# POZAlabs/ComMU-code

Measured on AMD Instinct MI355X. Metric: training tokens/sec at d_model=512 tgt_len=1024, higher is better.
Workload: dtype bf16; 1 GPU; transformer-xl train step L6 D512 H8 DI1024 tgt_len1024 mem_len0 vocab729; global_batch=64, batch_per_gpu=64, batch_chunk=1, seq_len=1024, parallelism=dp1, optimizer=clip1.0+Adam+invsqrt-LR, launch=eager, weights=random init (train.py:291-342)

## Files before the change

commu-code_amd/commu_amd/_lib.py:

```python
from __future__ import annotations

import ctypes as C
import os

_HERE = os.path.dirname(os.path.abspath(__file__))
LIB_PATH = os.path.join(os.path.dirname(_HERE), "lib", "libcommu_hip.so")

c_p = C.c_void_p
c_i = C.c_int
c_f = C.c_float
c_z = C.c_size_t


class AttnDesc(C.Structure):
    _fields_ = [("q", c_p), ("k", c_p), ("v", c_p), ("rd", c_p), ("r_w_bias", c_p), ("r_r_bias", c_p),
                ("reset", c_p), ("ld_qkv", c_i), ("ld_rd", c_i), ("ld_o", c_i), ("T", c_i), ("M", c_i),
                ("B", c_i), ("H", c_i), ("DH", c_i), ("same_length", c_i), ("sshift", c_i), ("scale", c_f),
                ("drop_p", c_f), ("drop_seed", C.c_uint)]


class AttnBwdDesc(C.Structure):
    _fields_ = [("dout", c_p), ("lse", c_p), ("delta", c_p), ("qu2", c_p), ("qv2", c_p), ("dq_ac", c_p),
                ("dk", c_p), ("dv", c_p), ("dsk", c_p), ("du_part", c_p), ("ld_dqkv", c_i), ("ld_dsk", c_i),
                ("du_rows", c_i), ("dsk_wedge", c_i), ("dsk_tiled", c_i), ("p_scratch", c_p), ("o", c_p), ("pf", c_p)]
# ... 36 lines not shown

class DecodeLoopArgs(C.Structure):
    _fields_ = [("struct_bytes", C.c_uint),
                ("logits", c_p), ("wrong", c_p), ("ld", c_i), ("V", c_i), ("B", c_i),
                ("temperature_rows", c_p), ("top_k_rows", c_p), ("top_p_rows", c_p),
                ("temperature", c_f), ("top_k", c_i), ("top_p", c_f),
                ("token", c_p), ("probs_out", c_p), ("logp", c_p), ("seq_logp", c_p), ("ldp", c_i),
                ("state", c_p), ("seq", c_p), ("chord_tok", c_p), ("chord_pos", c_p), ("utable", c_p),
                ("ld_seq", c_i), ("ld_chord", c_i), ("ld_u", c_i), ("max_iters", c_i),
                ("tok", c_p), ("active", c_p), ("keep", c_p), ("draw", c_p), ("uni", c_p), ("trace", c_p), ("ld_trace", c_i),
                ("klen", c_p), ("lmax", c_i),
                ("bias", c_p), ("gram", c_p), ("gram_on", c_p), ("harm", c_p), ("harm_on", c_p),
                ("ld_bias", c_i), ("ld_gram", c_i), ("ld_harm", c_i),
                ("cls_ctl", c_p)]


def struct_args(cls, **fields):
    return cls(struct_bytes=C.sizeof(cls), **fields)


PROTOTYPES = {
    "commu_gemm_nt_bf16": [c_p, c_i, c_p, c_i, c_p, c_i, c_i, c_i, c_i, c_p, c_p, c_i, c_p, c_i, c_i, C.c_uint, c_f, c_f, c_p],
    "commu_gemm_nt_signbits_words": [c_i, c_i, c_i, c_i, c_i, c_i],
    "commu_gemm_nt_ln_bf16": [c_p, c_i, c_p, c_p, c_i, c_f, c_p, c_i, c_p, c_i, c_p, c_i, c_i, c_i, c_i, c_p, c_p, c_i, c_i, c_p],
    "commu_gemm_tn_bf16": [c_p, c_i, c_p, c_i, c_p, c_i, c_z, c_i, c_i, c_i, c_i, c_i, c_p],
    "commu_gemm_nt_bf16_batched": [c_p, c_i, C.c_longlong, c_p, c_i, C.c_longlong, c_p, c_i, C.c_longlong, c_i, c_i,
                                   c_i, c_p, c_i, C.c_longlong, c_i, c_i, c_i, c_i, c_p],
    "commu_gemm_tn_slices": [c_i, c_i, c_i],
    "commu_gemm_tn_bf16_batched": [c_p, c_i, C.c_longlong, c_p, c_i, C.c_longlong, c_p, c_i, c_z, c_i, c_i, c_i, c_i,
                                   c_i, c_i, c_i, c_p],
    "commu_gemm_tn_grouped_slices": [C.POINTER(TnProblem), c_i, c_i],
    "commu_gemm_tn_grouped_slices_budget": [C.POINTER(TnProblem), c_i, c_i, c_i],
    "commu_gemm_tn_bf16_grouped": [C.POINTER(TnProblem), c_i, c_i, c_p, C.c_longlong, c_i, c_p],
    "commu_reduce_slabs2d_f32": [c_p, c_i, C.c_longlong, c_p, c_i, c_i, c_i, c_z, c_i, c_i, c_f, c_p],
    "commu_reduce_slabs_f32": [c_p, c_p, c_z, c_i, c_z, c_i, c_f, c_p],
    "commu_quant_mxfp8": [c_p, c_i, c_p, c_i, c_p, c_i, c_i, c_i, c_p],
    "commu_gemm_nt_mxfp8": [c_p, c_i, c_p, c_i, c_p, c_i, c_p, c_i, c_p, c_i, c_i, c_i, c_i, c_p, c_p, c_i, c_i, C.c_uint, c_f, c_p],
    "commu_reduce_slabs_group_f32": [C.POINTER(ReduceItem), c_i, c_p, c_i, c_z, c_i, c_f, c_p],
    "commu_reduce_slabs_crop_f32": [c_p, c_p, c_i, c_i, c_i, c_i, c_i, c_i, c_i, c_z, c_i, c_f, c_p],
    "commu_embed_fwd": [c_p, c_p, c_p, c_i, c_i, c_i, c_i, c_f, C.c_uint, c_f, c_p],
    "commu_embed_bwd": [c_p, c_p, c_i, c_p, c_i, c_i, c_i, c_f, c_i, C.c_uint, c_f, c_p],
    "commu_embed_bwd_ws_rows": [c_i, c_i],
    "commu_embed_bwd_sorted": [c_p, c_p, c_p, c_i, c_p, c_i, c_i, c_i, c_p, c_f, c_i, C.c_uint, c_f, c_p],
    "commu_posemb_fwd": [c_p, c_p, c_i, c_i, c_i, c_i, C.c_uint, c_f, c_p],
    "commu_layernorm_fwd": [c_p, c_i, c_p, c_p, c_p, c_i, c_p, c_p, c_i, c_i, c_f, c_p, c_i, C.c_uint, c_f, c_p],
    "commu_layernorm_bwd_nblocks": [c_i],
# ... 84 lines not shown
    "commu_embed_f32": [c_p, c_p, c_p, c_i, c_i, c_i, c_f, c_p],
    "commu_posemb_f32": [c_p, c_p, c_i, c_i, c_i, c_i, c_p],
    "commu_relattn_f32": [c_p, c_i, c_p, c_p, C.c_longlong, C.c_longlong, c_p, c_i, c_p, c_p, c_p, c_p, c_p, c_i, c_i, c_i,
                          c_i, c_i, c_i, c_i, c_i, c_f, c_p],
    "commu_decode_kv_append_f32": [c_p, c_i, c_p, c_p, c_p, c_p, c_i, c_i, c_i, c_p],
    "commu_decode_kv_append_ring_f32": [c_p, c_i, c_p, c_p, c_p, c_p, c_i, c_i, c_i, c_p],
    "commu_decode_attn_ring_f32": [c_p, c_i, c_p, c_p, c_p, c_i, c_p, c_p, c_p, c_p, c_i, c_i, c_i, c_i, c_i, c_i, c_f, c_p],
    "commu_gemm_f32": [c_i, c_i, c_p, c_i, c_p, c_i, c_p, c_i, c_i, c_i, c_i, c_p, c_i, c_f, C.c_uint, c_p, c_i, c_i, c_p, c_i,
                       c_p],
    "commu_relattn_fwd_f32": [c_p, c_i, c_p, c_p, c_i, c_p, c_i, c_p, c_p, c_p, c_p, c_i, c_p, c_i, c_i, c_i, c_i, c_i, c_i, c_i,
                              c_f, c_f, C.c_uint, c_p],
    "commu_relattn_bwd_f32": [c_p, c_i, c_p, c_p, c_i, c_p, c_i, c_p, c_p, c_p, c_p, c_i, c_p, c_i, c_p, c_p, c_p, c_i, c_p, c_p,
                              c_p, c_p, c_i, c_p, c_i, c_i, c_i, c_i, c_i, c_i, c_i, c_i, c_f, c_f, C.c_uint, c_p],
    "commu_layernorm_fwd_f32": [c_p, c_i, c_p, c_p, c_p, c_i, c_p, c_p, c_i, c_i, c_f, c_p],
    "commu_layernorm_bwd_f32": [c_p, c_i, c_p, c_i, c_p, c_i, c_p, c_p, c_p, c_p, c_i, c_p, c_i, c_p, c_p, c_i, c_i, c_p],
    "commu_ce_bwd_f32": [c_p, c_i, c_p, c_p, c_p, c_p, c_i, c_i, c_i, c_p],
    "commu_embed_bwd_f32": [c_p, c_p, c_p, c_i, c_p, c_i, c_i, c_f, c_f, C.c_uint, c_p],
    "commu_dropout_f32": [c_p, c_i, c_p, c_i, c_p, c_i, c_i, c_i, c_f, C.c_uint, c_p],
    "commu_hip_version": [],
}
_RESTYPE = {"commu_decode_tail_pack_bytes": C.c_longlong, "commu_attn_pf_bytes": C.c_longlong, "commu_hip_version": C.c_char_p, "commu_attn_p_scratch_elems": C.c_longlong,
            "commu_gemm_nt_signbits_words": C.c_longlong, "commu_pack_batch": C.c_longlong}
_NOCHECK = {"commu_layernorm_bwd_nblocks", "commu_colsum_slabs", "commu_embed_bwd_ws_rows", "commu_hip_version", "commu_attn_bwd_qrows", "commu_attn_fwd_generation", "commu_attn_bwd_kv_generation", "commu_colsum_slab_pass", "commu_gemm_tn_grouped_slices", "commu_gemm_tn_grouped_slices_budget", "commu_attn_band_slabs", "commu_attn_band_pairs",
            "commu_forcing_state_ints", "commu_decode_tail_supported", "commu_decode_tail_sync_words", "commu_decode_tail_sync_words_for", "commu_decode_tail_pack_bytes", "commu_attn_p_scratch_elems", "commu_gemm_nt_signbits_words", "commu_pack_batch", "commu_attn_pf_bytes",
            "commu_decode_prefix_chunk", "commu_decode_prefix_group", "commu_sample_args_bytes", "commu_decode_loop_args_bytes"}

_lib = None


class CommuHipError(RuntimeError):
    pass


def load():
    global _lib
    if _lib is not None:
        return _lib
    if not os.path.exists(LIB_PATH):
        raise CommuHipError(
            f"{LIB_PATH} not found: build it with `python commu-code_amd/build.py` "
            "(the product path has no CPU fallback)")
    import torch
    lib = C.CDLL(LIB_PATH)
    for name, argtypes in PROTOTYPES.items():
        fn = getattr(lib, name)
        fn.argtypes = argtypes
        fn.restype = _RESTYPE.get(name, c_i)
# ... 48 lines not shown
```

commu-code_amd/commu_amd/model/model.py:

```python
from __future__ import annotations

import math
from typing import List, Optional

import torch
import torch.nn as nn

from .. import ops
from .._lib import CommuHipError

BF16, F32 = torch.bfloat16, torch.float32
VPAD = 768


def _no_direct_forward(self, *a, **kw):
    raise CommuHipError(f"{type(self).__name__} is a parameter holder; call MemTransformerLM.forward")


class AdaptiveEmbedding(nn.Module):

    def __init__(self, n_token, d_embed, d_proj):
        super().__init__()
        if d_proj != d_embed:
            raise CommuHipError("d_proj != d_embed is dead code in the reference and is not built")
# ... 665 lines not shown
            f8 = self._weights_fp8(i) if fp8 else None
            if M > 0:
                cat = mems[i].reshape(M * B, D)
                if cat.dtype != BF16:
                    cat = cat.to(BF16)
                if fp8:
                    ops.linear_mxfp8(cat, (f8["qkv"][0][HD:], f8["qkv"][1][HD:]), out=qkv[:M * B, HD:])
                else:
                    ops.gemm_nt(cat, w["qkv"][HD:], out=qkv[:M * B, HD:])
            if fp8:
                ops.linear_mxfp8(h, f8["qkv"], out=qkv[M * B:])
            else:
                ops.gemm_nt(h, w["qkv"], out=qkv[M * B:])
            rd = rd_all[i] if rd_all is not None else ops.gemm_nt(pd, w["r"])
            vec, lse, qs = ops.relattn_fwd(qkv[M * B:, :HD], qkv[:, HD:2 * HD], qkv[:, 2 * HD:], rd, u, vb, rst,
                                           T, M, B, H, DH, bool(self.same_length), int(self.mem_len),
                                           save_q=need_grad, save_p=need_grad, drop_p=patt, drop_seed=ss(s0),
                                           scale=self.attn_scale)
            lin = (lambda x, k, **e: ops.linear_mxfp8(x, f8[k], **e)) if fp8 else (lambda x, k, **e: ops.gemm_nt(x, w[k], **e))
            z1 = lin(vec, "o", resid=h, drop_p=p, drop_seed=ss(s0 + 1))
            a, mu1, rs1 = ops.layernorm_fwd(z1, lay[i].dec_attn.layer_norm.weight, lay[i].dec_attn.layer_norm.bias)
            hbits = None
            if need_grad and not fp8 and not gelu and getattr(self, "relu_sign_bits", True):
                nw = ops.signbits_words(TB, DI, D, a.stride(0), w["w1"].stride(0), DI)
                if nw > 0 and ops.signbits_words(TB, DI, D, D, D, DI) > 0:
                    hbits = torch.empty(nw, device=dev, dtype=torch.int32)
            zff = None
            if gelu:
                zff = ops.gemm_nt(a, w["w1"], bias=w["b1"])
                hid = ops.gelu_fwd(zff, drop_p=p, drop_seed=ss(s0 + 2))
            elif hbits is not None:
                hid = ops.gemm_nt(a, w["w1"], bias=w["b1"], relu=True, drop_p=p, drop_seed=ss(s0 + 2), sign_bits_out=hbits)
            else:
                hid = lin(a, "w1", bias=w["b1"], relu=True, drop_p=p, drop_seed=ss(s0 + 2))
            z2 = lin(hid, "w2", bias=w["b2"], resid=a, drop_p=p, drop_seed=ss(s0 + 3))
            if i == L - 1 and p > 0:
                h_out = torch.empty(TB, D, device=dev, dtype=BF16)
            y, mu2, rs2 = ops.layernorm_fwd(z2, lay[i].pos_ff.layer_norm.weight, lay[i].pos_ff.layer_norm.bias,
                                            y=hids[i + 1], y_drop=h_out, drop_p=p, drop_seed=ss(2))
            if need_grad:
                sv.h.append(h); sv.cat.append(cat); sv.qkv.append(qkv); sv.rd.append(rd); sv.vec.append(vec)
                sv.lse.append(lse); sv.qs.append(qs); sv.z1.append(z1); sv.mu1.append(mu1); sv.rs1.append(rs1)
                sv.a.append(a); sv.hid.append(hid); sv.hbits.append(hbits); sv.zff.append(zff); sv.z2.append(z2)
                sv.mu2.append(mu2); sv.rs2.append(rs2)
            if want_kv:
                kv_out.append(qkv)
            h = y
        if h_out is None:
            h_out = h
# ... 161 lines not shown

        dy_add = None
        for i in range(L - 1, -1, -1):
            pre = f"layers.{i}."
            lay = self.layers[i]
            s0 = 16 + 4 * i
            if i == 0 and side is not None:
                side_mark[0] = torch.cuda.Event()
                side_mark[0].record(side)
            dz2m = torch.empty(TB, D, device=dev, dtype=BF16) if p > 0 else None
            dz2, part = ops.layernorm_bwd(dy, sv.z2[i], sv.mu2[i], sv.rs2[i], lay.pos_ff.layer_norm.weight,
                                          dz_masked=dz2m, drop_p=p, drop_seed=ss(s0 + 3), add=dy_add)
            dy_add = None
            if dz2m is None:
                dz2m = dz2
            keep.append(part)
            light(lambda part=part, pre=pre: ops.layernorm_bwd_reduce(
                part, gv(pre + "pos_ff.layer_norm.weight", (Dt,)), gv(pre + "pos_ff.layer_norm.bias", (Dt,)),
                gv(pre + "pos_ff.CoreNet.3.bias", (Dt,)), group=cgrp))
            wgrad(dz2m, sv.hid[i], gv(pre + "pos_ff.CoreNet.3.weight", (Dt, DIt)), crop=spec("w2"))
            hb = sv.hbits[i]
            if sv.zff[i] is not None:
                dhid = ops.gelu_bwd(ops.gemm_nt(dz2m, sh[f"w2_t{i}"]), sv.zff[i], drop_p=p, drop_seed=ss(s0 + 2))
            elif hb is not None and ops.signbits_words(TB, DI, D, dz2m.stride(0), sh[f"w2_t{i}"].stride(0), DI) == hb.numel():
                dhid = ops.gemm_nt(dz2m, sh[f"w2_t{i}"], relu_bits=hb, mask_scale=inv_keep)
            else:
                dhid = ops.gemm_nt(dz2m, sh[f"w2_t{i}"], relu_mask=sv.hid[i], mask_scale=inv_keep)
            wgrad(dhid, sv.a[i], gv(pre + "pos_ff.CoreNet.0.weight", (DIt, Dt)), crop=spec("w1"),
                  colsum=(gv(pre + "pos_ff.CoreNet.0.bias", (DIt,)), DIt))
            rln = bool(getattr(self, "resid_in_ln_bwd", False))
            da = ops.gemm_nt(dhid, sh[f"w1_t{i}"]) if rln else ops.gemm_nt(dhid, sh[f"w1_t{i}"], resid=dz2)
            dz1m = torch.empty(TB, D, device=dev, dtype=BF16) if p > 0 else None
            dz1, part = ops.layernorm_bwd(da, sv.z1[i], sv.mu1[i], sv.rs1[i], lay.dec_attn.layer_norm.weight,
                                          dz_masked=dz1m, drop_p=p, drop_seed=ss(s0 + 1), add=dz2 if rln else None)
            if dz1m is None:
                dz1m = dz1
            keep.append(part)
            light(lambda part=part, pre=pre: ops.layernorm_bwd_reduce(
                part, gv(pre + "dec_attn.layer_norm.weight", (Dt,)), gv(pre + "dec_attn.layer_norm.bias", (Dt,)), group=cgrp))
            wgrad(dz1m, sv.vec[i], gv(pre + "dec_attn.o_net.weight", (Dt, HDt)), crop=spec("o"))
            last = i == 0
            hook_last = last and cgrp is None and side is not None
            if last:
                flush_wgrads()
            dvec = ops.gemm_nt(dz1m, sh[f"o_t{i}"])
            qkv = sv.qkv[i]
            dqkv = torch.empty(K * B, 3 * HD, device=dev, dtype=BF16)
# ... 129 lines not shown
```

commu-code_amd/commu_amd/ops.py:

```python
from __future__ import annotations

import ctypes as C
import math
from typing import Optional

import torch

from . import _lib
from ._lib import AttnBwdDesc, AttnDesc, CommuHipError, call

EPI_BIAS, EPI_RELU, EPI_RESID, EPI_RELUMASK, EPI_OUT_F32, EPI_DROPOUT, EPI_SIGNBITS_OUT, EPI_RELUBITS = 1, 2, 4, 8, 16, 32, 64, 128


def site_seed(base_seed: int, site: int) -> int:
    x = (base_seed * 0x9E3779B9 + site * 0x85EBCA6B + 0x165667B1) & 0xFFFFFFFF
    x ^= x >> 16
    x = (x * 0x7feb352d) & 0xFFFFFFFF
    x ^= x >> 15
    x = (x * 0x846ca68b) & 0xFFFFFFFF
    x ^= x >> 16
    return x


def _mix32(x):
# ... 90 lines not shown
def attn_bwd_kv_generation(gen: int) -> int:
    return call("commu_attn_bwd_kv_generation", int(gen))


def _rowmajor2d(t: torch.Tensor, name: str):
    if t.dim() != 2 or t.stride(1) != 1:
        raise ValueError(f"{name}: need a 2-D tensor with unit column stride, got {tuple(t.shape)} / {t.stride()}")
    return t.stride(0)


def gemm_nt_layers(A, Bflat, N, K, stride, batch, out=None):
    M = A.shape[0]
    assert A.dtype == BF16 and Bflat.dtype == BF16 and A.shape[1] == K and Bflat.is_contiguous()
    assert Bflat.numel() >= (batch - 1) * stride + N * K
    if out is None:
        out = torch.empty(batch, M, N, device=A.device, dtype=BF16)
    call("commu_gemm_nt_bf16_batched", _p(A), _rowmajor2d(A, "A"), 0, _p(Bflat), K, stride, _p(out), N, M * N, M, N, K,
         None, 0, 0, 0, batch, 0, 0, _s())
    return out


def signbits_words(M, N, K, lda=None, ldb=None, ldc=None):
    return int(call("commu_gemm_nt_signbits_words", M, N, K, K if lda is None else lda, K if ldb is None else ldb,
                    N if ldc is None else ldc))


def gemm_nt(A, B, out=None, *, bias=None, resid=None, relu=False, relu_mask=None, out_f32=False,
            drop_p=0.0, drop_seed=0, mask_scale=1.0, sign_bits_out=None, relu_bits=None):
    lda, ldb = _rowmajor2d(A, "A"), _rowmajor2d(B, "B")
    M, K = A.shape
    N = B.shape[0]
    assert B.shape[1] == K and A.dtype == BF16 and B.dtype == BF16
    if out is None:
        out = torch.empty(M, N, device=A.device, dtype=F32 if out_f32 else BF16)
    ldc = _rowmajor2d(out, "out")
    flags = 0
    if bias is not None:
        flags |= EPI_BIAS
        assert bias.dtype == F32 and bias.numel() >= N
    if resid is not None:
        flags |= EPI_RESID
        assert resid.dtype == BF16
    if relu:
        flags |= EPI_RELU
    if relu_mask is not None:
        flags |= EPI_RELUMASK
# ... 1193 lines not shown
```

commu-code_amd/csrc/capi.hip:

```cpp
#include "commu_hip.h"
#include <hip/hip_runtime.h>
extern "C" const char* commu_hip_version(void) { return "commu_hip 0.1 (gfx950)"; }

int commu_seed_salt_elementwise(const unsigned*, hipStream_t);
int commu_seed_salt_relattn(const unsigned*, hipStream_t);
int commu_seed_salt_gemm(const unsigned*, hipStream_t);
int commu_seed_salt_gemm8(const unsigned*, hipStream_t);
int commu_seed_salt_gemm_fp8(const unsigned*, hipStream_t);

extern "C" int commu_set_seed_salt(const unsigned* src, hipStream_t stream) {
    int rc = commu_seed_salt_elementwise(src, stream);
    if (rc == 0) rc = commu_seed_salt_relattn(src, stream);
    if (rc == 0) rc = commu_seed_salt_gemm(src, stream);
    if (rc == 0) rc = commu_seed_salt_gemm8(src, stream);
    if (rc == 0) rc = commu_seed_salt_gemm_fp8(src, stream);
    return rc;
}
```

commu-code_amd/csrc/gemm.hip:

```cpp
#include "common.h"
#include "commu_hip.h"
#include "gemm8.h"
#include <math.h>
#include <stdlib.h>

namespace {

constexpr int BK = 32;

__device__ __forceinline__ int swz64(int row) { return ((row >> 3) & 1) * 3; }

struct GemmBatch {
    long long a, b, c, r;
    int tri_B, tri_M;
};

template <int BKT>
__device__ __forceinline__ int swzk(int row) { return BKT == 64 ? (row & 7) : swz64(row); }

template <int NBW>
__device__ __forceinline__ int colperm(int r) {
    const int c = r & 15, ni = (r >> 4) & (NBW - 1);
    if (NBW == 4) return (r & ~63) + 32 * (ni >> 1) + 8 * (c >> 2) + 4 * (ni & 1) + (c & 3);
    return (r & ~31) + 8 * (c >> 2) + 4 * ni + (c & 3);
}
// ... 522 lines not shown
            f32x4* o = (f32x4*)(dp + (size_t)r * ldd + c);
            *o = (accumulate ? *o : (f32x4){0.f, 0.f, 0.f, 0.f}) + alpha * s;
        }
        return;
    }
    for (size_t i = (size_t)blockIdx.x * blockDim.x + threadIdx.x; i < n; i += (size_t)gridDim.x * blockDim.x) {
        float s = 0.f;
        for (int k = 0; k < nslabs; ++k) s += sp[(size_t)k * stride + i];
        const int r = (int)((unsigned)i / (unsigned)cols), c = (int)((unsigned)i - (unsigned)r * (unsigned)cols);
        float* o = dp + (size_t)r * ldd + c;
        *o = (accumulate ? *o : 0.f) + alpha * s;
    }
}

}

static int launch_gemm_nt(const void* A, int lda, const void* B, int ldb, void* C, int ldc, int M, int N, int K,
                          const float* bias, const void* resid, int ldr, const void* relu_mask, int ldm, int flags,
                          unsigned drop_seed, float drop_p, float mask_scale, int batch, GemmBatch bs,
                          hipStream_t stream, const SkinnyLN* ln = nullptr) {
    if (M <= 0 || N <= 0 || batch <= 0) return 0;
    if (K <= 0 || (K % 32) != 0 || (lda % 8) || (ldb % 8) || (ldc % 4)) return -22;
    if (flags & (COMMU_EPI_SIGNBITS_OUT | COMMU_EPI_RELUBITS)) {
        if (batch != 1 || ln != nullptr || relu_mask == nullptr || !gemm8_nt_bits_eligible(M, N, K, lda, ldb, ldc, flags))
            return -22;
        G8Args g8{(const bf16*)A, (const bf16*)B, C, lda, ldb, ldc, M, N, K, (M + 255) / 256, (N + 255) / 256,
                  bias, nullptr, 0, (const bf16*)relu_mask, 0, flags, drop_seed,
                  drop_threshold16(drop_p), drop_keep_scale16(drop_threshold16(drop_p)), mask_scale, 0, nullptr};
        return launch_gemm8_nt(g8, stream);
    }
    const bool skinny = M <= 64 && batch == 1 && bs.tri_B == 0 && (K % 128) == 0 && K <= 1024 && N >= 32 &&
                        !(flags & (COMMU_EPI_DROPOUT | COMMU_EPI_RELUMASK));
    if (ln != nullptr && !skinny) return -22;
    if (skinny && (ln != nullptr || !getenv("COMMU_GEMM_NOSKINNY"))) {
        dim3 grid((N + 31) / 32);
#define SK_LAUNCH(KS, NWV)                                                                                           \
    {                                                                                                                \
        if (ln != nullptr) {                                                                                         \
            if (flags & COMMU_EPI_OUT_F32)                                                                           \
                COMMU_LAUNCH((gemm_nt_skinny_kernel<KS, true, NWV, true>), grid, dim3(64 * NWV), 0, stream,          \
                             (const bf16*)A, lda, (const bf16*)B, ldb, C, ldc, M, N, bias, (const bf16*)resid, ldr,  \
                             flags, *ln);                                                                            \
            else                                                                                                     \
                COMMU_LAUNCH((gemm_nt_skinny_kernel<KS, false, NWV, true>), grid, dim3(64 * NWV), 0, stream,         \
                             (const bf16*)A, lda, (const bf16*)B, ldb, C, ldc, M, N, bias, (const bf16*)resid, ldr,  \
                             flags, *ln);                                                                            \
        } else if (flags & COMMU_EPI_OUT_F32)                                                                        \
            COMMU_LAUNCH((gemm_nt_skinny_kernel<KS, true, NWV>), grid, dim3(64 * NWV), 0, stream, (const bf16*)A,    \
// ... 2 lines not shown
            COMMU_LAUNCH((gemm_nt_skinny_kernel<KS, false, NWV>), grid, dim3(64 * NWV), 0, stream, (const bf16*)A,   \
                         lda, (const bf16*)B, ldb, C, ldc, M, N, bias, (const bf16*)resid, ldr, flags, SkinnyLN{});  \
    }
        if (K % 256 == 0 && K >= 768) {
            switch (K / 256) {
                case 3: SK_LAUNCH(3, 8) break;
                default: SK_LAUNCH(4, 8) break;
            }
        } else {
            switch (K / 128) {
                case 1: SK_LAUNCH(1, 4) break;
                case 2: SK_LAUNCH(2, 4) break;
                case 3: SK_LAUNCH(3, 4) break;
                case 4: SK_LAUNCH(4, 4) break;
                case 5: SK_LAUNCH(5, 4) break;
                case 6: SK_LAUNCH(6, 4) break;
                case 7: SK_LAUNCH(7, 4) break;
                default: SK_LAUNCH(8, 4) break;
            }
        }
#undef SK_LAUNCH
        COMMU_LAUNCH_CHECK();
        return 0;
    }
    if (gemm8_nt_eligible(M, N, K, lda, ldb, batch, bs.tri_B, flags)) {
        G8Args g8{(const bf16*)A, (const bf16*)B, C, lda, ldb, ldc, M, N, K, (M + 255) / 256, (N + 255) / 256,
                  bias, (const bf16*)resid, ldr, (const bf16*)relu_mask, ldm, flags, drop_seed,
                  drop_threshold16(drop_p), drop_keep_scale16(drop_threshold16(drop_p)), mask_scale, 0, nullptr};
        return launch_gemm8_nt(g8, stream);
    }
    const bool narrow = (N <= 64);
    const bool large = !narrow && M >= 2048 && N >= 128 && !getenv("COMMU_GEMM_SMALL");
    const bool big = large && N >= 1024 && (N % 256 == 0) && !getenv("COMMU_GEMM_TALL");
    const bool tall = large && !big;
    const int bn = narrow ? 64 : (tall ? 128 : (big ? 256 : 128)), bm = (big || tall) ? 256 : 128;
    const int tiles_m = (M + bm - 1) / bm, tiles_n = (N + bn - 1) / bn;
    dim3 grid(tiles_m * tiles_n, batch);
    const unsigned drop_thr = drop_threshold16(drop_p);
    const float drop_scale = drop_keep_scale16(drop_thr);
#define NT_LAUNCH(F32, NBW, BKT)                                                                                   \
    COMMU_LAUNCH((gemm_nt_kernel<F32, NBW, BKT>), grid, dim3(256), 0, stream, (const bf16*)A, lda, (const bf16*)B, \
                 ldb, C, ldc, M, N, K, bias, (const bf16*)resid, ldr, (const bf16*)relu_mask, ldm, flags,          \
                 tiles_n, drop_seed, drop_thr, drop_scale, mask_scale, bs)
    const bool k64 = (K % 64 == 0) && !getenv("COMMU_GEMM_BK32");
    if (tall) {
        if (flags & COMMU_EPI_OUT_F32)
// ... 5 lines not shown
                         (const bf16*)B, ldb, C, ldc, M, N, K, bias, (const bf16*)resid, ldr, (const bf16*)relu_mask,
                         ldm, flags, tiles_n, drop_seed, drop_thr, drop_scale, mask_scale, bs);
    } else if (big) {
        if (flags & COMMU_EPI_OUT_F32)
            COMMU_LAUNCH((gemm_nt_kernel<true, 4, 32, 8, 2, 4>), grid, dim3(512), 0, stream, (const bf16*)A, lda,
                         (const bf16*)B, ldb, C, ldc, M, N, K, bias, (const bf16*)resid, ldr, (const bf16*)relu_mask,
                         ldm, flags, tiles_n, drop_seed, drop_thr, drop_scale, mask_scale, bs);
        else
            COMMU_LAUNCH((gemm_nt_kernel<false, 4, 32, 8, 2, 4>), grid, dim3(512), 0, stream, (const bf16*)A, lda,
                         (const bf16*)B, ldb, C, ldc, M, N, K, bias, (const bf16*)resid, ldr, (const bf16*)relu_mask,
                         ldm, flags, tiles_n, drop_seed, drop_thr, drop_scale, mask_scale, bs);
    } else if (flags & COMMU_EPI_OUT_F32) {
        if (narrow) { if (k64) NT_LAUNCH(true, 2, 64); else NT_LAUNCH(true, 2, 32); }
        else { if (k64) NT_LAUNCH(true, 4, 64); else NT_LAUNCH(true, 4, 32); }
    } else {
        if (narrow) { if (k64) NT_LAUNCH(false, 2, 64); else NT_LAUNCH(false, 2, 32); }
        else { if (k64) NT_LAUNCH(false, 4, 64); else NT_LAUNCH(false, 4, 32); }
    }
#undef NT_LAUNCH
    COMMU_LAUNCH_CHECK();
    return 0;
}

extern "C" long long commu_gemm_nt_signbits_words(int M, int N, int K, int lda, int ldb, int ldc) {
    if (M <= 0 || N <= 0 || !gemm8_nt_bits_eligible(M, N, K, lda, ldb, ldc, 0)) return 0;
    return (long long)M * N / 32;
}

extern "C" int commu_gemm_nt_bf16(const void* A, int lda, const void* B, int ldb, void* C, int ldc,
                                  int M, int N, int K, const float* bias, const void* resid, int ldr,
                                  const void* relu_mask, int ldm, int flags, unsigned drop_seed, float drop_p,
                                  float mask_scale, hipStream_t stream) {
    return launch_gemm_nt(A, lda, B, ldb, C, ldc, M, N, K, bias, resid, ldr, relu_mask, ldm, flags, drop_seed, drop_p,
                          mask_scale, 1, GemmBatch{0, 0, 0, 0, 0, 0}, stream);
}

extern "C" int commu_gemm_nt_bf16_batched(const void* A, int lda, long long strideA, const void* B, int ldb,
                                          long long strideB, void* C, int ldc, long long strideC, int M, int N,
                                          int K, const void* resid, int ldr, long long strideR, int flags,
                                          int batch, int tri_B, int tri_M, hipStream_t stream) {
    return launch_gemm_nt(A, lda, B, ldb, C, ldc, M, N, K, nullptr, resid, ldr, nullptr, 0, flags, 0u, 0.f, 1.f, batch,
                          GemmBatch{strideA, strideB, strideC, strideR, tri_B, tri_M}, stream);
}

static int tn_tile(int M, int N, int K) {
    if (K <= 64) return 0;
    if (N >= 256 && K >= 256 && M >= 8192 && !getenv("COMMU_TN_SMALL")) return 2;
    return 1;
// ... 244 lines not shown
```

include/commu_hip.h:

```cpp
#ifndef COMMU_HIP_H
#define COMMU_HIP_H

#include <stddef.h>
#include <stdint.h>

#ifndef __HIP_PLATFORM_AMD__
typedef struct ihipStream_t* hipStream_t;
#endif

#ifdef __cplusplus
extern "C" {
#endif

enum {
    COMMU_EPI_BIAS = 1,
    COMMU_EPI_RELU = 2,
    COMMU_EPI_RESID = 4,
    COMMU_EPI_RELUMASK = 8,
    COMMU_EPI_OUT_F32 = 16,
    COMMU_EPI_DROPOUT = 32,
    COMMU_EPI_SIGNBITS_OUT = 64,
    COMMU_EPI_RELUBITS = 128
};
long long commu_gemm_nt_signbits_words(int M, int N, int K, int lda, int ldb, int ldc);
int commu_gemm_nt_bf16(const void* A, int lda, const void* B, int ldb, void* C, int ldc, int M, int N,
                       int K, const float* bias, const void* resid, int ldr, const void* relu_mask,
                       int ldm, int flags, unsigned drop_seed, float drop_p, float mask_scale,
                       hipStream_t stream);
int commu_gemm_nt_ln_bf16(const void* z, int ldz, const float* gamma, const float* beta, int D, float eps,
                          void* a_out, int lda_out, const void* B, int ldb, void* C, int ldc, int M, int N, int K,
                          const float* bias, const void* resid, int ldr, int flags, hipStream_t stream);
int commu_gemm_nt_bf16_batched(const void* A, int lda, long long strideA, const void* B, int ldb,
                               long long strideB, void* C, int ldc, long long strideC, int M, int N, int K,
                               const void* resid, int ldr, long long strideR, int flags, int batch,
                               int tri_B, int tri_M, hipStream_t stream);
int commu_gemm_tn_bf16(const void* A, int lda, const void* B, int ldb, float* slabs, int ldc,
                       size_t slab_stride, int M, int N, int K, int nslices, int mode, hipStream_t stream);
int commu_gemm_tn_slices(int M, int N, int K);
int commu_gemm_tn_bf16_batched(const void* A, int lda, long long strideA, const void* B, int ldb,
                               long long strideB, float* slabs, int ldc, size_t slab_stride, int M, int N, int K,
                               int nslices, int batch, int tri_B, int tri_M, hipStream_t stream);
typedef struct commu_tn_problem {
    const void* A;
    const void* B;
    int lda, ldb, N, K;
    long long out_off;
    long long colsum_off;
// ... 369 lines not shown
```

Baseline: 4.384 million tokens/s.

## Add persistent weight-stationary bf16 GEMM kernel for K=512 with fused epilogues

Adds a persistent NT GEMM kernel for K=512 and N a multiple of 512. Each workgroup keeps a 128-column weight slab in registers and streams 128-row A tiles through an 8-stage LDS ring filled by buffer-load-to-LDS DMA. Blocks are mapped to row blocks with an XCD-aware schedule, and the kernel fuses residual-add, dropout, bias+ReLU with sign-bit output, and relu-bit masking epilogues. By default it handles only the residual and residual+dropout forms at M≥16384, which covers the attention output projection here. It adds a signbits-family query so the saved ReLU bit layout matches the kernel that produced it. The aim is to cut weight reloads and improve load/MFMA overlap, at the cost of heavy register use and an inline-asm pipeline that is hard to maintain.

After: 4.382 million tokens/s (median of 2 runs). Within noise of the previous version (-0.1%).

```diff
diff --git a/commu-code_amd/commu_amd/_lib.py b/commu-code_amd/commu_amd/_lib.py
--- a/commu-code_amd/commu_amd/_lib.py
+++ b/commu-code_amd/commu_amd/_lib.py
@@ -82,6 +82,7 @@
 PROTOTYPES = {
     "commu_gemm_nt_bf16": [c_p, c_i, c_p, c_i, c_p, c_i, c_i, c_i, c_i, c_p, c_p, c_i, c_p, c_i, c_i, C.c_uint, c_f, c_f, c_p],
     "commu_gemm_nt_signbits_words": [c_i, c_i, c_i, c_i, c_i, c_i],
+    "commu_gemm_signbits_family": [c_i, c_i, c_i, c_i, c_i, c_i],
     "commu_gemm_nt_ln_bf16": [c_p, c_i, c_p, c_p, c_i, c_f, c_p, c_i, c_p, c_i, c_p, c_i, c_i, c_i, c_i, c_p, c_p, c_i, c_i, c_p],
     "commu_gemm_tn_bf16": [c_p, c_i, c_p, c_i, c_p, c_i, c_z, c_i, c_i, c_i, c_i, c_i, c_p],
     "commu_gemm_nt_bf16_batched": [c_p, c_i, C.c_longlong, c_p, c_i, C.c_longlong, c_p, c_i, C.c_longlong, c_i, c_i,
@@ -212,7 +213,7 @@
 _RESTYPE = {"commu_decode_tail_pack_bytes": C.c_longlong, "commu_attn_pf_bytes": C.c_longlong, "commu_hip_version": C.c_char_p, "commu_attn_p_scratch_elems": C.c_longlong,
             "commu_gemm_nt_signbits_words": C.c_longlong, "commu_pack_batch": C.c_longlong}
 _NOCHECK = {"commu_layernorm_bwd_nblocks", "commu_colsum_slabs", "commu_embed_bwd_ws_rows", "commu_hip_version", "commu_attn_bwd_qrows", "commu_attn_fwd_generation", "commu_attn_bwd_kv_generation", "commu_colsum_slab_pass", "commu_gemm_tn_grouped_slices", "commu_gemm_tn_grouped_slices_budget", "commu_attn_band_slabs", "commu_attn_band_pairs",
-            "commu_forcing_state_ints", "commu_decode_tail_supported", "commu_decode_tail_sync_words", "commu_decode_tail_sync_words_for", "commu_decode_tail_pack_bytes", "commu_attn_p_scratch_elems", "commu_gemm_nt_signbits_words", "commu_pack_batch", "commu_attn_pf_bytes",
+            "commu_forcing_state_ints", "commu_decode_tail_supported", "commu_decode_tail_sync_words", "commu_decode_tail_sync_words_for", "commu_decode_tail_pack_bytes", "commu_attn_p_scratch_elems", "commu_gemm_nt_signbits_words", "commu_gemm_signbits_family", "commu_pack_batch", "commu_attn_pf_bytes",
             "commu_decode_prefix_chunk", "commu_decode_prefix_group", "commu_sample_args_bytes", "commu_decode_loop_args_bytes"}
 
 _lib = None
diff --git a/commu-code_amd/commu_amd/model/model.py b/commu-code_amd/commu_amd/model/model.py
--- a/commu-code_amd/commu_amd/model/model.py
+++ b/commu-code_amd/commu_amd/model/model.py
@@ -711,9 +711,10 @@
             a, mu1, rs1 = ops.layernorm_fwd(z1, lay[i].dec_attn.layer_norm.weight, lay[i].dec_attn.layer_norm.bias)
             hbits = None
             if need_grad and not fp8 and not gelu and getattr(self, "relu_sign_bits", True):
-                nw = ops.signbits_words(TB, DI, D, a.stride(0), w["w1"].stride(0), DI)
-                if nw > 0 and ops.signbits_words(TB, DI, D, D, D, DI) > 0:
-                    hbits = torch.empty(nw, device=dev, dtype=torch.int32)
+                fam = ops.gemm_signbits_family(TB, DI, D, a.stride(0), w["w1"].stride(0), DI)
+                if fam != 0 and ops.gemm_signbits_family(TB, DI, D, D, D, DI) == fam:
+                    hbits = torch.empty(TB * DI // 32, device=dev, dtype=torch.int32)
+                    self._relu_bits_family = fam
             zff = None
             if gelu:
                 zff = ops.gemm_nt(a, w["w1"], bias=w["b1"])
@@ -921,7 +922,8 @@
             hb = sv.hbits[i]
             if sv.zff[i] is not None:
                 dhid = ops.gelu_bwd(ops.gemm_nt(dz2m, sh[f"w2_t{i}"]), sv.zff[i], drop_p=p, drop_seed=ss(s0 + 2))
-            elif hb is not None and ops.signbits_words(TB, DI, D, dz2m.stride(0), sh[f"w2_t{i}"].stride(0), DI) == hb.numel():
+            elif hb is not None and ops.gemm_signbits_family(TB, DI, D, dz2m.stride(0), sh[f"w2_t{i}"].stride(0), DI) == \
+                    getattr(self, "_relu_bits_family", 0):
                 dhid = ops.gemm_nt(dz2m, sh[f"w2_t{i}"], relu_bits=hb, mask_scale=inv_keep)
             else:
                 dhid = ops.gemm_nt(dz2m, sh[f"w2_t{i}"], relu_mask=sv.hid[i], mask_scale=inv_keep)
diff --git a/commu-code_amd/commu_amd/ops.py b/commu-code_amd/commu_amd/ops.py
--- a/commu-code_amd/commu_amd/ops.py
+++ b/commu-code_amd/commu_amd/ops.py
@@ -136,6 +136,11 @@
 
 def signbits_words(M, N, K, lda=None, ldb=None, ldc=None):
     return int(call("commu_gemm_nt_signbits_words", M, N, K, K if lda is None else lda, K if ldb is None else ldb,
+                    N if ldc is None else ldc))
+
+
+def gemm_signbits_family(M, N, K, lda=None, ldb=None, ldc=None):
+    return int(call("commu_gemm_signbits_family", M, N, K, K if lda is None else lda, K if ldb is None else ldb,
                     N if ldc is None else ldc))
 
 
diff --git a/commu-code_amd/csrc/capi.hip b/commu-code_amd/csrc/capi.hip
--- a/commu-code_amd/csrc/capi.hip
+++ b/commu-code_amd/csrc/capi.hip
@@ -7,6 +7,7 @@
 int commu_seed_salt_gemm(const unsigned*, hipStream_t);
 int commu_seed_salt_gemm8(const unsigned*, hipStream_t);
 int commu_seed_salt_gemm_fp8(const unsigned*, hipStream_t);
+int commu_seed_salt_gemm_ws(const unsigned*, hipStream_t);
 
 extern "C" int commu_set_seed_salt(const unsigned* src, hipStream_t stream) {
     int rc = commu_seed_salt_elementwise(src, stream);
@@ -14,5 +15,6 @@
     if (rc == 0) rc = commu_seed_salt_gemm(src, stream);
     if (rc == 0) rc = commu_seed_salt_gemm8(src, stream);
     if (rc == 0) rc = commu_seed_salt_gemm_fp8(src, stream);
+    if (rc == 0) rc = commu_seed_salt_gemm_ws(src, stream);
     return rc;
 }
diff --git a/commu-code_amd/csrc/gemm.hip b/commu-code_amd/csrc/gemm.hip
--- a/commu-code_amd/csrc/gemm.hip
+++ b/commu-code_amd/csrc/gemm.hip
@@ -1,6 +1,7 @@
 #include "common.h"
 #include "commu_hip.h"
 #include "gemm8.h"
+#include "gemm_ws.h"
 #include <math.h>
 #include <stdlib.h>
 
@@ -569,8 +570,14 @@
     if (M <= 0 || N <= 0 || batch <= 0) return 0;
     if (K <= 0 || (K % 32) != 0 || (lda % 8) || (ldb % 8) || (ldc % 4)) return -22;
     if (flags & (COMMU_EPI_SIGNBITS_OUT | COMMU_EPI_RELUBITS)) {
-        if (batch != 1 || ln != nullptr || relu_mask == nullptr || !gemm8_nt_bits_eligible(M, N, K, lda, ldb, ldc, flags))
-            return -22;
+        if (batch != 1 || ln != nullptr || relu_mask == nullptr) return -22;
+        if (gemm_ws_bits_take(M, N, K, lda, ldb, ldc)) {
+            if (!gemm_ws_takes(M, N, K, lda, ldb, ldc, ldr, flags, batch, bs.tri_B)) return -22;
+            WsArgs ws{(const bf16*)A, (const bf16*)B, (bf16*)C, lda, ldb, ldc, M, N, bias, nullptr, 0, (unsigned*)relu_mask,
+                      flags, drop_seed, drop_threshold16(drop_p), drop_keep_scale16(drop_threshold16(drop_p)), mask_scale};
+            return launch_gemm_ws(ws, stream);
+        }
+        if (!gemm8_nt_bits_eligible(M, N, K, lda, ldb, ldc, flags)) return -22;
         G8Args g8{(const bf16*)A, (const bf16*)B, C, lda, ldb, ldc, M, N, K, (M + 255) / 256, (N + 255) / 256,
                   bias, nullptr, 0, (const bf16*)relu_mask, 0, flags, drop_seed,
                   drop_threshold16(drop_p), drop_keep_scale16(drop_threshold16(drop_p)), mask_scale, 0, nullptr};
@@ -619,6 +626,11 @@
 #undef SK_LAUNCH
         COMMU_LAUNCH_CHECK();
         return 0;
+    }
+    if (gemm_ws_takes(M, N, K, lda, ldb, ldc, ldr, flags, batch, bs.tri_B)) {
+        WsArgs ws{(const bf16*)A, (const bf16*)B, (bf16*)C, lda, ldb, ldc, M, N, bias, (const bf16*)resid, ldr, nullptr,
+                  flags, drop_seed, drop_threshold16(drop_p), drop_keep_scale16(drop_threshold16(drop_p)), mask_scale};
+        return launch_gemm_ws(ws, stream);
     }
     if (gemm8_nt_eligible(M, N, K, lda, ldb, batch, bs.tri_B, flags)) {
         G8Args g8{(const bf16*)A, (const bf16*)B, C, lda, ldb, ldc, M, N, K, (M + 255) / 256, (N + 255) / 256,
@@ -670,8 +682,14 @@
     return 0;
 }
 
+extern "C" int commu_gemm_signbits_family(int M, int N, int K, int lda, int ldb, int ldc) {
+    if (M <= 0 || N <= 0) return 0;
+    if (gemm_ws_bits_take(M, N, K, lda, ldb, ldc)) return 2;
+    return gemm8_nt_bits_eligible(M, N, K, lda, ldb, ldc, 0) ? 1 : 0;
+}
+
 extern "C" long long commu_gemm_nt_signbits_words(int M, int N, int K, int lda, int ldb, int ldc) {
-    if (M <= 0 || N <= 0 || !gemm8_nt_bits_eligible(M, N, K, lda, ldb, ldc, 0)) return 0;
+    if (commu_gemm_signbits_family(M, N, K, lda, ldb, ldc) == 0) return 0;
     return (long long)M * N / 32;
 }
 
diff --git a/commu-code_amd/csrc/gemm_ws.h b/commu-code_amd/csrc/gemm_ws.h
--- /dev/null
+++ b/commu-code_amd/csrc/gemm_ws.h
@@ -0,0 +1,39 @@
+#pragma once
+#include "common.h"
+
+struct WsArgs {
+    const bf16* A;
+    const bf16* B;
+    bf16* C;
+    int lda, ldb, ldc, M, N;
+    const float* bias;
+    const bf16* resid;
+    int ldr;
+    unsigned* bits;
+    int flags;
+    unsigned drop_seed, drop_thr;
+    float drop_scale, mask_scale;
+};
+
+struct WsMap {
+    int slab, first, stride, count;
+};
+__host__ __device__ inline WsMap ws_map(int nrb, int G, int bid) {
+    if ((G & 31) == 0) {
+        const int xcd = bid & 7, idx = bid >> 3, R = G >> 5;
+        const int slab = idx & 3, r = idx >> 2;
+        const int q8 = nrb >> 3, r8 = nrb & 7;
+        const int xbase = xcd < r8 ? xcd * (q8 + 1) : r8 * (q8 + 1) + (xcd - r8) * q8;
+        const int xcount = q8 + (xcd < r8 ? 1 : 0);
+        return WsMap{slab, xbase + r, R, r < xcount ? (xcount - r + R - 1) / R : 0};
+    }
+    const int slab = bid & 3, lane = bid >> 2, L = G >> 2;
+    return WsMap{slab, lane, L, lane < nrb ? (nrb - lane + L - 1) / L : 0};
+}
+
+enum { WS_FORM_PLAIN = 1, WS_FORM_BRD_BITS = 2, WS_FORM_RELUBITS = 4, WS_FORM_RESID = 8, WS_FORM_RESID_DROP = 16 };
+
+int gemm_ws_form(int flags);
+bool gemm_ws_takes(int M, int N, int K, int lda, int ldb, int ldc, int ldr, int flags, int batch, int tri_B);
+bool gemm_ws_bits_take(int M, int N, int K, int lda, int ldb, int ldc);
+int launch_gemm_ws(const WsArgs& a, hipStream_t stream);
diff --git a/commu-code_amd/csrc/gemm_ws.hip b/commu-code_amd/csrc/gemm_ws.hip
--- /dev/null
+++ b/commu-code_amd/csrc/gemm_ws.hip
@@ -0,0 +1,326 @@
+#include "gemm_ws.h"
+#include "commu_hip.h"
+#include <stdlib.h>
+
+namespace {
+
+typedef __amdgpu_buffer_rsrc_t srd_t;
+
+constexpr int WS_STAGE = 16384;
+constexpr int WS_NST = 8;
+constexpr int WS_D = 7;
+constexpr int WS_MIN_M = 16384;
+
+__device__ __forceinline__ void dma16(srd_t srd, unsigned voff, unsigned soff, unsigned lds_dst) {
+    asm volatile("s_mov_b32 m0, %0\n\ts_nop 0\n\tbuffer_load_dwordx4 %1, %2, %3 offen lds"
+                 :: "s"(lds_dst), "v"(voff), "s"(srd), "s"(soff) : "memory");
+}
+__device__ __forceinline__ void dma4(srd_t srd, unsigned voff, unsigned lds_dst) {
+    asm volatile("s_mov_b32 m0, %0\n\ts_nop 0\n\tbuffer_load_dword %1, %2, 0 offen lds"
+                 :: "s"(lds_dst), "v"(voff), "s"(srd) : "memory");
+}
+template <int N>
+__device__ __forceinline__ void ws_vmcnt() {
+    asm volatile("s_waitcnt vmcnt(%0)" :: "n"(N) : "memory");
+}
+
+#define WS_WAIT_LGKM() asm volatile("s_waitcnt lgkmcnt(0)" ::: "memory")
+#define WS_BAR()                               \
+    do {                                       \
+        __builtin_amdgcn_sched_barrier(0);     \
+        __builtin_amdgcn_s_barrier();          \
+        __builtin_amdgcn_sched_barrier(0);     \
+    } while (0)
+
+template <int AUX, bool BRELU, bool DROP, bool BITS_OUT>
+__global__ __launch_bounds__(512) void gemm_nt_ws_kernel(const WsArgs a) {
+    constexpr int AUX_BYTES = AUX == 1 ? 8 * 4096 : (AUX == 2 ? 8 * 256 : 16);
+    __shared__ __attribute__((aligned(1024))) char smem[WS_NST * WS_STAGE + AUX_BYTES];
+    constexpr int E = 4 + (BITS_OUT ? 1 : 0) + (AUX == 1 ? 4 : (AUX == 2 ? 1 : 0));
+    const int tid = threadIdx.x, lane = tid & 63;
+    const int w = __builtin_amdgcn_readfirstlane(tid >> 6);
+    const int wr = w >> 2, wc = w & 3, r16 = lane & 15, g = lane >> 4;
+    DropKey dk{0u, 0u};
+    if (DROP) {
+        dk = drop_key(salted(a.drop_seed));
+        dk.key = __builtin_amdgcn_readfirstlane(dk.key);
+        dk.k2 = __builtin_amdgcn_readfirstlane(dk.k2);
+        asm volatile("" : "+s"(dk.key), "+s"(dk.k2));
+    }
+
+    const int M = a.M, N = a.N;
+    const int nrb = (M + 127) >> 7, P = N >> 9;
+    const WsMap mp = ws_map(nrb, (int)gridDim.x, (int)blockIdx.x);
+    if (mp.count == 0) return;
+    const int nitems = mp.count * P;
+
+    unsigned voffX[2];
+#pragma unroll
+    for (int j = 0; j < 2; ++j) {
+        const int h = 16 * w + 8 * j + (lane >> 3);
+        const int c = (lane & 7) ^ ((h >> 1) & 7);
+        voffX[j] = (unsigned)(h * a.lda + c * 8) * 2u;
+    }
+    const unsigned lds0 = (unsigned)(size_t)(LDS_AS char*)smem;
+    const srd_t srdA = __builtin_amdgcn_make_buffer_rsrc((void*)a.A, 0, (int)(unsigned)(((size_t)(M - 1) * a.lda + 512) * 2), 0x00020000);
+    int s_rbi = 0, s_kt = 0, s_left = nitems;
+    auto stage_next = [&]() {
+        const unsigned m0 = (unsigned)(s_left > 0 ? mp.first + s_rbi * mp.stride : nrb) * 128u;
+        const unsigned soff = m0 * (unsigned)a.lda * 2u + (unsigned)s_kt * 128u;
+        const unsigned dst = lds0 + s_kt * WS_STAGE + w * 2048;
+        dma16(srdA, voffX[0], soff, dst);
+        dma16(srdA, voffX[1], soff, dst + 1024);
+        if (++s_kt == WS_NST) {
+            s_kt = 0;
+            --s_left;
+            if (++s_rbi == mp.count) s_rbi = 0;
+        }
+    };
+
+    const unsigned auxl = lds0 + WS_NST * WS_STAGE + w * (AUX == 1 ? 4096 : 256);
+    const LDS_AS char* auxp = (const LDS_AS char*)smem + WS_NST * WS_STAGE + w * (AUX == 1 ? 4096 : 256);
+    const srd_t srdR = __builtin_amdgcn_make_buffer_rsrc(
+        (void*)(AUX == 1 ? (const void*)a.resid : (const void*)a.bits), 0,
+        AUX == 1 ? (int)(unsigned)(((size_t)(M - 1) * a.ldr + N) * 2) : (AUX == 2 ? (int)(unsigned)((size_t)M * N / 8) : 0), 0x00020000);
+    auto aux_stage = [&](int rb, int ncol) {
+        if (AUX == 1) {
+            const unsigned vo = (unsigned)(r16 * a.ldr + 8 * g) * 2u;
+#pragma unroll
+            for (int mi = 0; mi < 4; ++mi) {
+                const unsigned so = ((unsigned)(rb * 128 + wr * 64 + 16 * mi) * (unsigned)a.ldr + (unsigned)ncol) * 2u;
+                dma16(srdR, vo, so, auxl + mi * 1024);
+            }
+        } else if (AUX == 2) {
+            dma4(srdR, (unsigned)(((rb * 2 + wr) * (N >> 5) + (ncol >> 5)) * 64 + lane) * 4u, auxl);
+        }
+    };
+
+    const LDS_AS char* lds = (const LDS_AS char*)smem;
+    const int laneoff = (r16 >> 3) * 1024 + (r16 & 7) * 128 + wr * 8192;
+    const int ch0 = (g ^ ((r16 >> 1) & 7)) << 4;
+    const int xo0 = laneoff + ch0, xo1 = laneoff + (ch0 ^ 64);
+#define WS_FRAG(off) (*(const LDS_AS bf16x8*)(lds + (off)))
+
+    f32x4 acc[2][4];
+#pragma unroll
+    for (int i = 0; i < 2; ++i)
+#pragma unroll
+        for (int j = 0; j < 4; ++j) acc[i][j] = (f32x4){0.f, 0.f, 0.f, 0.f};
+    bf16x8 wf[2][16];
+    float bv[8];
+#pragma unroll
+    for (int e = 0; e < 8; ++e) bv[e] = 0.f;
+    auto load_w = [&](int ncol) {
+#pragma unroll
+        for (int ni = 0; ni < 2; ++ni)
+#pragma unroll
+            for (int ks = 0; ks < 16; ++ks)
+                wf[ni][ks] = ld_bf16x8(a.B + (size_t)(ncol + 8 * (r16 >> 2) + 4 * ni + (r16 & 3)) * a.ldb + 32 * ks + 8 * g);
+        if (BRELU) {
+            const f32x4 b0 = *(const f32x4*)(a.bias + ncol + 8 * g), b1 = *(const f32x4*)(a.bias + ncol + 8 * g + 4);
+#pragma unroll
+            for (int e = 0; e < 4; ++e) { bv[e] = b0[e]; bv[4 + e] = b1[e]; }
+        }
+#pragma unroll
+        for (int ni = 0; ni < 2; ++ni)
+#pragma unroll
+            for (int ks = 0; ks < 16; ++ks) asm volatile("" : "+v"(wf[ni][ks]));
+#pragma unroll
+        for (int e = 0; e < 8; ++e) asm volatile("" : "+v"(bv[e]));
+    };
+
+    if (AUX) aux_stage(mp.first, mp.slab * 128 + wc * 32);
+#pragma unroll
+    for (int u = 0; u < WS_D; ++u) stage_next();
+    load_w(mp.slab * 128 + wc * 32);
+    ws_vmcnt<0>();
+    WS_BAR();
+    if (wr == 1) WS_BAR();
+    bf16x8 xa[4], xb[4];
+
+    bool adj = false;
+    int pass = 0, rbi = 0;
+    for (int item = 0; item < nitems; ++item) {
+        const int ncol = pass * 512 + mp.slab * 128 + wc * 32;
+        if (rbi == 0 && pass > 0) load_w(ncol);
+        const int rb = mp.first + rbi * mp.stride;
+#pragma unroll
+        for (int kt = 0; kt < WS_NST; ++kt) {
+            stage_next();
+#pragma unroll
+            for (int mi = 0; mi < 4; ++mi) {
+                xa[mi] = WS_FRAG(kt * WS_STAGE + xo0 + mi * 2048);
+                xb[mi] = WS_FRAG(kt * WS_STAGE + xo1 + mi * 2048);
+            }
+            if (kt < WS_D - 1 && adj) ws_vmcnt<2 * (WS_D - 1) + E>();
+            else ws_vmcnt<2 * (WS_D - 1)>();
+            WS_WAIT_LGKM();
+            WS_BAR();
+            __builtin_amdgcn_s_setprio(1);
+#pragma unroll
+            for (int ni = 0; ni < 2; ++ni)
+#pragma unroll
+                for (int mi = 0; mi < 4; ++mi) acc[ni][mi] = mfma16(wf[ni][2 * kt], xa[mi], acc[ni][mi]);
+#pragma unroll
+            for (int ni = 0; ni < 2; ++ni)
+#pragma unroll
+                for (int mi = 0; mi < 4; ++mi) acc[ni][mi] = mfma16(wf[ni][2 * kt + 1], xb[mi], acc[ni][mi]);
+            __builtin_amdgcn_s_setprio(0);
+            if (kt < WS_NST - 1) WS_BAR();
+        }
+
+        const int mw = rb * 128 + wr * 64;
+        const bool interior = mw + 64 <= M;
+        unsigned word = 0u, bits_in = 0u;
+        if (AUX == 2) bits_in = *(const LDS_AS unsigned*)(auxp + lane * 4);
+#pragma unroll
+        for (int mi = 0; mi < 4; ++mi) {
+            const int m = mw + 16 * mi + r16, n = ncol + 8 * g;
+            float v[8];
+#pragma unroll
+            for (int e = 0; e < 8; ++e) v[e] = acc[e >> 2][mi][e & 3];
+            if (BRELU) {
+#pragma unroll
+                for (int e = 0; e < 8; ++e) v[e] = fmaxf(v[e] + bv[e], 0.f);
+            }
+            if (DROP) {
+                const unsigned q0 = ((unsigned)m * (unsigned)N + (unsigned)n) >> 1, thr_hi = a.drop_thr << 16;
+#pragma unroll
+                for (int e2 = 0; e2 < 4; ++e2) {
+                    const unsigned hw = drop_word(q0 + (unsigned)e2, dk);
+                    v[2 * e2] = (unsigned short)hw >= (unsigned short)a.drop_thr ? v[2 * e2] * a.drop_scale : 0.f;
+                    v[2 * e2 + 1] = hw >= thr_hi ? v[2 * e2 + 1] * a.drop_scale : 0.f;
+                }
+            }
+            if (AUX == 1) {
+                const bf16x8 r = *(const LDS_AS bf16x8*)(auxp + mi * 1024 + lane * 16);
+#pragma unroll
+                for (int e = 0; e < 8; ++e) v[e] += bf2f(r[e]);
+            }
+            if (AUX == 2) {
+#pragma unroll
+                for (int e = 0; e < 8; ++e) {
+                    const int keep = __builtin_amdgcn_sbfe((int)bits_in, 8 * mi + e, 1);
+                    v[e] = __builtin_bit_cast(float, __builtin_bit_cast(int, v[e] * a.mask_scale) & keep);
+                }
+            }
+            bf16x8 o;
+#pragma unroll
+            for (int e = 0; e < 8; ++e) o[e] = f2bf(v[e]);
+            if (BITS_OUT) {
+#pragma unroll
+                for (int e = 0; e < 8; ++e) word |= (bf2f(o[e]) > 0.f ? 1u : 0u) << (8 * mi + e);
+            }
+            bf16* cp = a.C + (size_t)m * a.ldc + n;
+            if (interior) st_bf16x8(cp, o);
+            else if (m < M) st_bf16x8(cp, o);
+            acc[0][mi] = (f32x4){0.f, 0.f, 0.f, 0.f};
+            acc[1][mi] = (f32x4){0.f, 0.f, 0.f, 0.f};
+        }
+        if (BITS_OUT && interior) a.bits[(size_t)((rb * 2 + wr) * (N >> 5) + (ncol >> 5)) * 64 + lane] = word;
+        adj = interior;
+        if (++rbi == mp.count) {
+            rbi = 0;
+            ++pass;
+        }
+        if (AUX && item + 1 < nitems) aux_stage(mp.first + rbi * mp.stride, pass * 512 + mp.slab * 128 + wc * 32);
+        WS_BAR();
+    }
+    ws_vmcnt<0>();
+    if (wr == 0) WS_BAR();
+#undef WS_FRAG
+}
+
+}
+
+int gemm_ws_form(int flags) {
+    const int f = flags & ~COMMU_EPI_DROPOUT;
+    const bool drop = (flags & COMMU_EPI_DROPOUT) != 0;
+    if (flags == 0) return WS_FORM_PLAIN;
+    if (f == (COMMU_EPI_BIAS | COMMU_EPI_RELU | COMMU_EPI_SIGNBITS_OUT)) return WS_FORM_BRD_BITS;
+    if (flags == COMMU_EPI_RELUBITS) return WS_FORM_RELUBITS;
+    if (f == COMMU_EPI_RESID) return drop ? WS_FORM_RESID_DROP : WS_FORM_RESID;
+    return 0;
+}
+
+static int ws_forms_mask() {
+    if (const char* e = getenv("COMMU_GEMM_WS_FORMS")) return atoi(e);
+    return WS_FORM_RESID | WS_FORM_RESID_DROP;
+}
+
+static bool ws_shape_ok(int M, int N, int K, int lda, int ldb, int ldc) {
+    if (getenv("COMMU_GEMM_WS_OFF")) return false;
+    if (K != 512 || N <= 0 || (N % 512) != 0 || M < 128) return false;
+    if (M < WS_MIN_M && !getenv("COMMU_GEMM_WS_ALWAYS")) return false;
+    if ((lda % 8) || (ldb % 8) || (ldc % 8) || lda < 512 || ldb < 512 || ldc < N) return false;
+    if ((size_t)(M + 256) * lda * 2 >= 0xFFFF0000ull || (size_t)M * N >= 0xFFFF0000ull) return false;
+    return true;
+}
+
+bool gemm_ws_takes(int M, int N, int K, int lda, int ldb, int ldc, int ldr, int flags, int batch, int tri_B) {
+    if (batch != 1 || tri_B != 0) return false;
+    const int form = gemm_ws_form(flags);
+    if (form == 0 || !(form & ws_forms_mask())) return false;
+    if (!ws_shape_ok(M, N, K, lda, ldb, ldc)) return false;
+    if (flags & COMMU_EPI_RESID) {
+        if ((ldr % 8) || ldr < N || (size_t)(M + 256) * ldr * 2 >= 0xFFFF0000ull) return false;
+    }
+    if (flags & (COMMU_EPI_SIGNBITS_OUT | COMMU_EPI_RELUBITS)) return gemm_ws_bits_take(M, N, K, lda, ldb, ldc);
+    return true;
+}
+
+bool gemm_ws_bits_take(int M, int N, int K, int lda, int ldb, int ldc) {
+    const int both = WS_FORM_BRD_BITS | WS_FORM_RELUBITS;
+    if ((M % 128) != 0 || (ws_forms_mask() & both) != both) return false;
+    return ws_shape_ok(M, N, K, lda, ldb, ldc);
+}
+
+static int ws_grid() {
+    int grid = 256;
+    if (const char* e = getenv("COMMU_GEMM_WS_GRID")) {
+        const int gsz = atoi(e) & ~3;
+        if (gsz >= 4 && gsz < grid) grid = gsz;
+    }
+    return grid;
+}
+
+extern "C" int commu_gemm_ws_cover(int M, int N, int grid) {
+    if (M <= 0 || N <= 0 || (N % 512) != 0 || grid < 4 || (grid & 3)) return -1;
+    const int nrb = (M + 127) / 128;
+    unsigned char* seen = (unsigned char*)calloc((size_t)nrb * 4, 1);
+    int bad = 0;
+    for (int bid = 0; bid < grid && !bad; ++bid) {
+        const WsMap mp = ws_map(nrb, grid, bid);
+        if (mp.slab < 0 || mp.slab > 3 || mp.count < 0) { bad = -2; break; }
+        for (int i = 0; i < mp.count; ++i) {
+            const int rb = mp.first + i * mp.stride;
+            if (rb < 0 || rb >= nrb || seen[rb * 4 + mp.slab]++) { bad = -2; break; }
+        }
+    }
+    for (int i = 0; i < nrb * 4 && !bad; ++i)
+        if (seen[i] != 1) bad = 1 + i;
+    free(seen);
+    return bad;
+}
+
+int launch_gemm_ws(const WsArgs& a, hipStream_t stream) {
+    const int grid = ws_grid();
+    const bool drop = (a.flags & COMMU_EPI_DROPOUT) != 0;
+#define WS_LAUNCH(AUX, BR, DR, BO) COMMU_LAUNCH((gemm_nt_ws_kernel<AUX, BR, DR, BO>), dim3(grid), dim3(512), 0, stream, a)
+    switch (gemm_ws_form(a.flags)) {
+        case WS_FORM_PLAIN: WS_LAUNCH(0, false, false, false); break;
+        case WS_FORM_BRD_BITS:
+            if (drop) WS_LAUNCH(0, true, true, true);
+            else WS_LAUNCH(0, true, false, true);
+            break;
+        case WS_FORM_RELUBITS: WS_LAUNCH(2, false, false, false); break;
+        case WS_FORM_RESID: WS_LAUNCH(1, false, false, false); break;
+        case WS_FORM_RESID_DROP: WS_LAUNCH(1, false, true, false); break;
+        default: return -22;
+    }
+#undef WS_LAUNCH
+    COMMU_LAUNCH_CHECK();
+    return 0;
+}
+
+COMMU_DEFINE_SEED_SALT_SETTER(commu_seed_salt_gemm_ws)
diff --git a/include/commu_hip.h b/include/commu_hip.h
--- a/include/commu_hip.h
+++ b/include/commu_hip.h
@@ -23,6 +23,7 @@
     COMMU_EPI_RELUBITS = 128
 };
 long long commu_gemm_nt_signbits_words(int M, int N, int K, int lda, int ldb, int ldc);
+int commu_gemm_signbits_family(int M, int N, int K, int lda, int ldb, int ldc);
 int commu_gemm_nt_bf16(const void* A, int lda, const void* B, int ldb, void* C, int ldc, int M, int N,
                        int K, const float* bias, const void* resid, int ldr, const void* relu_mask,
                        int ldm, int flags, unsigned drop_seed, float drop_p, float mask_scale,
```
